# anand-12/botorch

Hardware: AMD Instinct MI355X
Metric: acq-evals/sec (q x restarts x MC), qEI forward (higher is better)
Workload: dtype f64; 1 GPU; C3 qEI forward: SingleTaskGP n=4096 d=6, q=16, 512 restarts/GPU, 512 Sobol MC samples, best_f = max(Y) - 1.5; n=4096, d=6, q=16, restarts_per_gpu=512, mc=512, parallelism=restart-sharded x1

## Files before the change

botorch_amd/_lib.py:

```python
from __future__ import annotations

import ctypes
import os
from ctypes import POINTER, c_double, c_int, c_int64, c_void_p

_HERE = os.path.dirname(os.path.abspath(__file__))
LIB_PATH = os.path.join(_HERE, "libbotorch_amd.so")

BO_OK, BO_ERR_ARG, BO_ERR_HIP, BO_ERR_NOT_PSD, BO_ERR_NAN = 0, 1, 2, 3, 4
RBF, MATERN52 = 0, 1
GEMM_LOWER_C, GEMM_A_LOWER, GEMM_B_UPPER, GEMM_A_UPPER, GEMM_B_LOWER = 1, 2, 4, 8, 16
QMC_POSTERIOR, QMC_QEI, QMC_QNEI, QMC_CHOL, QMC_QLOGEI, QMC_QLOGNEI = 0, 1, 2, 3, 4, 5
QMC_QSR, QMC_QPI, QMC_QUCB = 6, 7, 8
LOG_MODES = (QMC_QLOGEI, QMC_QLOGNEI)
MC_MODES = (QMC_QEI, QMC_QNEI) + LOG_MODES + (QMC_QSR, QMC_QPI, QMC_QUCB)
ABI_VERSION = 12
RT_ROWMAJOR, RT_BLOCKED = 0, 1

_P = c_void_p

_SIGNATURES = {
    "bo_last_error": (ctypes.c_char_p, []),
    "bo_version": (c_int, []),
    "bo_probe_mfma_f64_layout": (c_int, [_P, _P]),
# ... 48 lines not shown
    "bo_post_w_members_work": (c_int, [c_int, c_int, c_int, c_int64, POINTER(c_int64)]),
    "bo_post_w_split_members": (c_int, [c_int, _P, c_int64, _P, c_int, c_int, c_int64, _P, _P, _P]),
    "bo_post_w_dx_work": (c_int, [c_int, c_int, c_int64, POINTER(c_int64)]),
    "bo_post_w_dx": (c_int, [c_int, _P, c_int64, _P, c_int, c_int, c_int, c_int64, _P, _P, _P, _P,
                             _P, _P, c_double, c_double, _P, _P, _P]),
    "bo_ainv": (c_int, [_P, c_int64, c_int64, _P, _P, _P]),
    "bo_sym_lower": (c_int, [_P, c_int64, c_int64, _P]),
    "bo_post_kxt_rows": (c_int, [c_int, _P, c_int, c_int, c_int, _P, _P, c_int64, c_double, _P,
                                 _P, _P]),
    "bo_post_quad_plan": (c_int, [c_int64, c_int, c_int64, POINTER(c_int)]),
    "bo_post_small_plan": (c_int, [c_int64, c_int, c_int64, POINTER(c_int)]),
    "bo_post_set_wide": (c_int, [c_int]),
    "bo_post_wide_applies": (c_int, [c_int64, c_int, c_int64, c_int, c_int, c_int, POINTER(c_int)]),
    "bo_post_wide_schedule": (c_int, [c_int, c_int, c_int, c_int, POINTER(c_int), POINTER(c_int),
                                      _P]),
    "bo_post_small": (c_int, [_P, c_int64, c_int, c_int64, _P, c_int64, _P, _P, _P, _P, _P]),
    "bo_post_small_batched": (c_int, [c_int, _P, _P, _P, _P, _P, _P, c_int64, c_int, c_int64,
                                      c_int64, _P]),
    "bo_pinned_alloc": (c_int, [c_int64, POINTER(c_void_p), POINTER(c_void_p)]),
    "bo_pinned_free": (c_int, [c_void_p]),
    "bo_qmc_finalize_members": (c_int, [c_int, c_int, c_int, c_int, _P, _P, _P, c_int64, _P, _P, _P,
                                        _P, c_int, c_double, _P, _P, _P, _P, c_int, _P, _P, _P,
                                        c_int, c_int64, _P, c_int64, _P]),
    "bo_post_kxt_rows_members": (c_int, [c_int, c_int, _P, c_int, c_int, c_int, _P, _P, _P, c_int64,
                                         _P, _P, _P]),
    "bo_post_members_work": (c_int, [c_int, c_int64, c_int, c_int64, POINTER(c_int64)]),
    "bo_post_partials_members": (c_int, [c_int, _P, _P, _P, _P, _P, _P, _P, c_int64, c_int,
                                         c_int64, c_int64, _P, _P]),
    "bo_post_quad": (c_int, [_P, _P, c_int64, _P, c_int64, c_int, c_int64, _P, _P, _P]),
    "bo_post_split_table": (c_int, [c_int64, c_int, c_int64, c_int, _P, c_int, _P, c_int,
# ... 231 lines not shown
    "bo_qmc_feas_v": QmcFeasArgs, "bo_qmc_feas_backward_v": QmcFeasArgs,
    "bo_kg_v": KgArgs, "bo_kg_backward_v": KgArgs,
    "bo_paths_eval_v": PathsArgs, "bo_paths_eval_backward_v": PathsArgs,
    "bo_jes_v": JesArgs, "bo_jes_backward_v": JesArgs,
    "bo_mes_v": MesArgs, "bo_mes_backward_v": MesArgs,
    "bo_gibbon_v": GibbonArgs, "bo_gibbon_backward_v": GibbonArgs,
    "bo_mv_quantiles_v": MvQuantilesArgs,
    "bo_nipv_gram_v": NipvArgs, "bo_nipv_gram_backward_v": NipvArgs,
    "bo_bald_v": BaldArgs, "bo_bald_backward_v": BaldArgs,
    "bo_analytic_v": AnalyticArgs, "bo_analytic_backward_v": AnalyticArgs,
    "bo_saas_potential_v": SaasPotentialArgs,
    "bo_lbfgs_step_v": LbfgsStepArgs, "bo_lbfgsb_step_v": LbfgsbArgs,
}
for _name, _cls in RECORD_ENTRIES.items():
    _SIGNATURES[_name] = (c_int, [POINTER(_cls), _P])
_SIGNATURES["bo_saas_potential_work"] = (c_int, [c_int64, c_int, c_int64, POINTER(c_int64)])
_SIGNATURES["bo_struct_size"] = (c_int64, [ctypes.c_char_p])
_SIGNATURES["bo_post_backward_jobs"] = (c_int, [c_int, POINTER(POINTER(PostBackwardArgs)), _P, _P])
ARG_RECORDS = {"BoPostPartialsArgs": PostPartialsArgs, "BoQmcFinalizeArgs": QmcFinalizeArgs,
               "BoQmcBackwardArgs": QmcBackwardArgs, "BoPostBackwardArgs": PostBackwardArgs,
               "BoQehviArgs": QehviArgs, "BoQehviFeasArgs": QehviFeasArgs,
               "BoQlogehviArgs": QlogehviArgs, "BoQmcFeasArgs": QmcFeasArgs, "BoKgArgs": KgArgs,
               "BoPathsArgs": PathsArgs, "BoJesArgs": JesArgs, "BoMesArgs": MesArgs,
               "BoGibbonArgs": GibbonArgs, "BoMvQuantilesArgs": MvQuantilesArgs,
               "BoNipvArgs": NipvArgs, "BoBaldArgs": BaldArgs, "BoAnalyticArgs": AnalyticArgs,
               "BoSaasPotentialArgs": SaasPotentialArgs,
               "BoLbfgsStepArgs": LbfgsStepArgs, "BoLbfgsbArgs": LbfgsbArgs}

_lib = None

# ... 62 lines not shown
```

botorch_amd/csrc/abi_structs.cpp:

```cpp
#include <cstdio>
#include <string>

#include "../../include/botorch_amd.h"

void bo_set_error(const char* fmt, ...);

namespace {

template <class T>
bool header_ok(const T* a, const char* name) {
  if (!a) {
    bo_set_error("%s: null argument struct", name);
    return false;
  }
  if (a->struct_size != sizeof(T) || a->abi_version != BO_ABI_VERSION) {
    bo_set_error("%s: struct size %u / ABI %u, library expects %zu / %d", name, a->struct_size,
                 a->abi_version, sizeof(T), BO_ABI_VERSION);
    return false;
  }
  return true;
}

}

// ... 35 lines not shown
  X(PostPartials) X(QmcFinalize) X(QmcBackward) X(PostBackward) X(Qehvi) X(QehviFeas)          \
  X(Qlogehvi) X(QmcFeas) X(Kg) X(Paths) X(Jes) X(Mes) X(Gibbon) X(MvQuantiles) X(Nipv) X(Bald) \
  X(Analytic) X(SaasPotential) X(LbfgsStep) X(Lbfgsb)

extern "C" {

#define BO_ENTRY(entry, record)                                         \
  int bo_##entry##_impl(const Bo##record##Args* a, void* stream);       \
  int bo_##entry##_v(const Bo##record##Args* a, void* stream) {         \
    if (!header_ok(a, "bo_" #entry "_v")) return BO_ERR_ARG;            \
    return bo_##entry##_impl(a, stream);                                \
  }
BO_RECORD_ENTRIES(BO_ENTRY)
#undef BO_ENTRY

int64_t bo_struct_size(const char* name) {
  const std::string s = name ? name : "";
#define BO_SIZE(record) \
  if (s == "Bo" #record "Args") return sizeof(Bo##record##Args);
  BO_RECORDS(BO_SIZE)
#undef BO_SIZE
  return -1;
}

}
```

botorch_amd/csrc/post.hip:

```cpp
#include "common.h"
#include "post_wide_sched.h"

#include <algorithm>
#include <atomic>
#include <cstdlib>
#include <map>
#include <mutex>
#include <tuple>
#include <vector>

namespace {

constexpr int PC = 128;
constexpr int PI = 128;
constexpr int PK = 16;
constexpr int PLD = 144;
constexpr int DP = 8;
constexpr int kSlots = 512;
constexpr int kTileDoubles = 32 * 64;
#ifndef KXT_K
#define KXT_K 16
#endif

template <int KIND, int ND>
// ... 553 lines not shown
      m += __shfl_xor(m, 16);
      m += __shfl_xor(m, 32);
      if (lane < 16) mpart[(int64_t)ci * nrows_pad + row0 + lane] = m;
    }
    }
  }
  }
}

#ifndef BO_POSTW_PRIO
#define BO_POSTW_PRIO 0
#endif
__global__ __launch_bounds__(512, 2) void post_partials_wide_kernel(
    int n, const double* __restrict__ U, int64_t ldu, const double* __restrict__ beta, int nC,
    int nI, double* __restrict__ Spart, double* __restrict__ mpart, double* __restrict__ Rt,
    const double* __restrict__ Kt, int rt_blk) {
  constexpr int SS = postw::kSS, NU = postw::kNU;
  __shared__ __attribute__((aligned(16))) double Us[postw::kStages][SS * PK][PLD];
  const int bid = blockIdx.x;
  const int xcd = bid & 7;
  const int slot = bid >> 3;
  const int tt = (slot >> 5) * 8 + xcd;
  const int w = slot & 31;
  const int nIG = nI >> 3;
  const int p = tt / nIG;
  if (p >= (nC >> 4)) return;
  const int ci_long = ((nC >> 3) - 1 - p) * 8 + 7 - (w & 7);
  const int ci_short = p * 8 + (w & 7);
  const int i0 = ((tt % nIG) * 4 + (w >> 3)) * (2 * PI);
  const int tid = threadIdx.x;
  const int lane = tid & 63;
  const int wave = __builtin_amdgcn_readfirstlane(tid >> 6);
  const bool late = postw::kLag > 0 && wave >= 4;
#if BO_POSTW_PRIO
  if (__builtin_amdgcn_readfirstlane(threadIdx.x) >= 256) __builtin_amdgcn_s_setprio(1);
#endif
  const int64_t ldk = (int64_t)nI * PI;
  const int nrows16 = nI * (PI / 16);
  const int lag = postw::lag_of(late);

  for (int sidx = 0; sidx < 2; ++sidx) {
    const int ci = sidx == 0 ? ci_long : ci_short;
    const int c0 = ci * PC;
    const int kend = min(n, c0 + PC);
// ... 152 lines not shown
          const int c = c0 + ct * 16 + mfma_row(lane, r);
          m = fma(acc[ct][it][r], (c < n) ? beta[c] : 0.0, m);
        }
      m += __shfl_xor(m, 16);
      m += __shfl_xor(m, 32);
      if (lane < 16) mpart[(int64_t)ci * nrows_pad + row0 + lane] = m;
    }
  }
}

struct RowsFromX {
  const double* X;
  const double* ls;
  int B, q, d, Qp;
  double* Xq_out;
};

struct KxtMembers {
  const double* ls[8];
  const double* Xt[8];
  double os[8];
  double* Xq[8];
  double* Kt[8];
  int nm;
};

template <int KIND, int ND, int KK = KXT_K, bool FROMX = false>
__global__ __launch_bounds__(256) void kxt_build_kernel(const double* __restrict__ Xq, int nrows,
                                                        const double* __restrict__ Xt, int n,
                                                        int np, int nrows_pad, double outputscale,
                                                        double* __restrict__ Kt,
                                                        RowsFromX rx = RowsFromX{},
                                                        KxtMembers km = KxtMembers{}) {
  if (km.nm > 0) {
    const int m = blockIdx.z;
    rx.ls = km.ls[m];
    rx.Xq_out = km.Xq[m];
    Xt = km.Xt[m];
    outputscale = km.os[m];
    Kt = km.Kt[m];
  }
  const int i = blockIdx.x * 256 + threadIdx.x;
  const int k0 = blockIdx.y * KK;
  const bool iv = i < nrows;
  double xi[ND];
  if constexpr (FROMX) {
    const int b = i / rx.Qp, a = i - (i / rx.Qp) * rx.Qp;
    const bool real = iv && b < rx.B && a < rx.q;
#pragma unroll
    for (int t = 0; t < ND; ++t)
      xi[t] = (real && t < rx.d) ? rx.X[((int64_t)b * rx.q + a) * rx.d + t] / rx.ls[t] : 0.0;
    if (blockIdx.y == 0 && i < nrows_pad) {
#pragma unroll
      for (int t = 0; t < DP; ++t)
        rx.Xq_out[(int64_t)i * DP + t] =
            (real && t < rx.d) ? rx.X[((int64_t)b * rx.q + a) * rx.d + t] / rx.ls[t] : 0.0;
    }
  } else {
#pragma unroll
    for (int t = 0; t < ND; ++t) xi[t] = iv ? Xq[(int64_t)i * DP + t] : 0.0;
  }
  if (i >= nrows_pad) return;
#pragma unroll 4
  for (int kk = 0; kk < KK; ++kk) {
    const int k = k0 + kk;
    if (k < np) Kt[(int64_t)k * nrows_pad + i] = eval_kernel_row<KIND, ND>(xi, Xt, n, k, outputscale, iv);
  }
}

__global__ __launch_bounds__(256) void post_splitk_reduce_kernel(
    const double* __restrict__ work, const int4* __restrict__ red, int n, int nI,
    const double* __restrict__ beta_all, double* __restrict__ Spart_all,
    double* __restrict__ mpart_all, double* __restrict__ Rt_all, PostMembers pm = PostMembers{}) {
  __shared__ double part[3][32][64];
  const int4 r4 = red[blockIdx.x / (PI / 16)];
  const int sub = blockIdx.x % (PI / 16);
  const int ci = r4.x & 0xffffff, rt = r4.y * (PI / 16) + sub;
  const int mem = r4.x >> 24;
  const bool memb = pm.nm > 0;
  const double* beta = memb ? pm.beta[mem] : beta_all;
  double* Spart = memb ? pm.Spart[mem] : Spart_all;
// ... 363 lines not shown
#ifndef BO_POST_WIDE_DEFAULT
#define BO_POST_WIDE_DEFAULT 1
#endif
static std::atomic<int>& wide_mode() {
  static std::atomic<int> m{[] {
    const char* e = std::getenv("BO_POST_WIDE");
    const int v = e ? std::atoi(e) : 0;
    return v >= -1 && v <= 1 ? v : 0;
  }()};
  return m;
}
static bool wide_applies(int nC, int nI, int kc_len, bool cross, bool pre) {
  const int mode = wide_mode().load();
  if (mode < 0 || (mode == 0 && !BO_POST_WIDE_DEFAULT)) return false;
  return kc_len == 0 && !cross && pre && nI > 0 && nC % 16 == 0 && nI % 8 == 0 && paired_enabled();
}

struct SplitPlan {
  std::vector<int4> segs, red;
  std::vector<int> wg_off;
  int nchunks = 0, max_segs = 0;
  int64_t max_steps = 0;
};

static int sk_min_share() {
  static const int v = [] {
    const char* e = std::getenv("BO_SK_MIN_SHARE");
    const int x = e ? std::atoi(e) : 4;
    return x >= 1 ? x : 4;
  }();
// ... 420 lines not shown
  BO_CHECK_ARG(X && lengthscale && Xt_scaled && outputscale && Xq && Kt,
               "bo_post_kxt_rows_members: null pointer");
  KxtMembers km{};
  km.nm = nm;
  for (int m = 0; m < nm; ++m) {
    BO_CHECK_ARG(lengthscale[m] && Xt_scaled[m] && Xq[m] && Kt[m], "bo_post_kxt_rows_members: null buffer");
    km.ls[m] = lengthscale[m];
    km.Xt[m] = Xt_scaled[m];
    km.os[m] = outputscale[m];
    km.Xq[m] = Xq[m];
    km.Kt[m] = Kt[m];
  }
  const int np = nC * PC;
  const int nrows = B * Qp;
  hipStream_t st = as_stream(stream);
  const RowsFromX rx{X, lengthscale[0], B, q, d, Qp, Xq[0]};
  const bool small = ceil_div(nrows_pad, 256) * ceil_div(np, KXT_K) * nm < 1024;
  const int kk = small ? kxt_small_k() : KXT_K;
  const dim3 grid((unsigned)ceil_div(nrows_pad, 256), (unsigned)ceil_div(np, kk), (unsigned)nm);
#define BO_KXTM_K(KIND, ND, K)                                                                 \
  kxt_build_kernel<KIND, ND, K, true><<<grid, 256, 0, st>>>(nullptr, nrows, Xt_scaled[0], (int)n, \
                                                            np, nrows_pad, outputscale[0], Kt[0], rx, km)
#define BO_KXTM(KIND, ND)                  \
  switch (kk) {                            \
    case 1: BO_KXTM_K(KIND, ND, 1); break; \
    case 2: BO_KXTM_K(KIND, ND, 2); break; \
    case 4: BO_KXTM_K(KIND, ND, 4); break; \
    case 8: BO_KXTM_K(KIND, ND, 8); break; \
    default: BO_KXTM_K(KIND, ND, KXT_K); break; \
  }
#define BO_KXTM_D(KIND)                      \
// ... 6 lines not shown
    case 6: BO_KXTM(KIND, 6); break;         \
    default: BO_KXTM(KIND, 8); break;        \
  }
  if (kind == BO_RBF) {
    BO_KXTM_D(BO_RBF)
  } else {
    BO_KXTM_D(BO_MATERN52)
  }
#undef BO_KXTM_D
#undef BO_KXTM
#undef BO_KXTM_K
  BO_LAUNCH_CHECK();
  return BO_OK;
}

int bo_post_kxt_rows(int kind, const double* X, int B, int q, int d, const double* lengthscale,
                     const double* Xt_scaled, int64_t n, double outputscale, double* Xq, double* Kt,
                     void* stream) {
  BO_CHECK_ARG(kind == BO_RBF || kind == BO_MATERN52, "bad kernel kind %d", kind);
  BO_CHECK_ARG(d >= 1 && d <= DP, "fused posterior kernel supports 1 <= d <= %d", DP);
  int Qp, nrows_pad, nC;
  int s = bo_post_geometry(B, q, n, &Qp, &nrows_pad, &nC);
  if (s) return s;
  if (nrows_pad == 0) return BO_OK;
  BO_CHECK_ARG(X && lengthscale && Xt_scaled && Xq && Kt, "bo_post_kxt_rows: null buffer");
  const int np = nC * PC;
  const int nrows = B * Qp;
  hipStream_t st = as_stream(stream);
  const RowsFromX rx{X, lengthscale, B, q, d, Qp, Xq};
  const bool small = ceil_div(nrows_pad, 256) * ceil_div(np, KXT_K) < 1024;
  const int kk = small ? kxt_small_k() : KXT_K;
  const dim3 grid((unsigned)ceil_div(nrows_pad, 256), (unsigned)ceil_div(np, kk));
#define BO_KXTR_K(KIND, ND, K)                                                                 \
  kxt_build_kernel<KIND, ND, K, true><<<grid, 256, 0, st>>>(nullptr, nrows, Xt_scaled, (int)n,  \
                                                            np, nrows_pad, outputscale, Kt, rx)
#define BO_KXTR(KIND, ND)                  \
  switch (kk) {                            \
    case 1: BO_KXTR_K(KIND, ND, 1); break; \
    case 2: BO_KXTR_K(KIND, ND, 2); break; \
    case 4: BO_KXTR_K(KIND, ND, 4); break; \
    case 8: BO_KXTR_K(KIND, ND, 8); break; \
    default: BO_KXTR_K(KIND, ND, KXT_K); break; \
  }
#define BO_KXTR_D(KIND)                      \
  switch (d) {                               \
    case 1: BO_KXTR(KIND, 1); break;         \
    case 2: BO_KXTR(KIND, 2); break;         \
    case 3: BO_KXTR(KIND, 3); break;         \
    case 4: BO_KXTR(KIND, 4); break;         \
    case 5: BO_KXTR(KIND, 5); break;         \
    case 6: BO_KXTR(KIND, 6); break;         \
    default: BO_KXTR(KIND, 8); break;        \
  }
  if (kind == BO_RBF) {
    BO_KXTR_D(BO_RBF)
  } else {
    BO_KXTR_D(BO_MATERN52)
  }
#undef BO_KXTR_D
#undef BO_KXTR
#undef BO_KXTR_K
  BO_LAUNCH_CHECK();
  return BO_OK;
}

int bo_post_partials_impl(const BoPostPartialsArgs* a, void* stream) {
  const int kc_len = a->kc_len;
  const int64_t n = a->n;
  const bool blocked = a->rt_layout == BO_RT_BLOCKED;
  BO_CHECK_ARG(a->rt_layout == BO_RT_ROWMAJOR || (blocked && kc_len == 0 && !a->Qc),
               "rt_layout %d: the blocked R^T is stored by one-pass grids without a cross term",
               a->rt_layout);
  BO_CHECK_ARG(a->Qc == nullptr || (kc_len == 0 && a->rq >= 1 && a->rq <= 16 && a->ldq >= n &&
                                    a->Cx != nullptr),
               "cross term: one-pass only, 1 <= rq <= 16 rows (got %d), ldq >= n, Cx given", a->rq);
  BO_CHECK_ARG(a->kind == BO_RBF || a->kind == BO_MATERN52, "bad kernel kind %d", a->kind);
  BO_CHECK_ARG(a->ldu % 2 == 0 && a->ldu >= ceil_div(n, PC) * PC, "U leading dim %lld too small",
               (long long)a->ldu);
  if (a->B == 0) return BO_OK;
  const bool pre = a->Kt != nullptr;
  BO_CHECK_ARG(kc_len == 0 || kc_len == -1 || (kc_len > 0 && kc_len % PK == 0),
// ... 9 lines not shown
                          ? ((nC % 16 == 0 && paired_enabled()) ? 2 : 1) : 0;
  DevPlan* plan = nullptr;
  if (kc_len != 0) {
    s = device_plan(nC, nI, (int)n, kc_len, &plan);
    if (s) return s;
    BO_CHECK_ARG(plan->nchunks == 0 || a->work != nullptr, "split plan needs a workspace of %lld doubles",
                 (long long)plan->nchunks * PI * PC);
  }
  const int64_t blocks = kc_len != 0    ? plan->W
                         : grouped == 2 ? 512 * (int64_t)ceil_div((nC / 16) * (nI / 8), 8)
                         : grouped      ? 512 * (int64_t)ceil_div((nC / 8) * (nI / 8), 8)
                                        : 8 * ceil_div(nC, 8) * (int64_t)nI;
  const int4* segs = plan ? plan->segs : nullptr;
  const int* wg_off = plan ? plan->wg_off : nullptr;
  hipStream_t st = as_stream(stream);
  if (wide_applies(nC, nI, kc_len, a->Qc != nullptr, pre)) {
    const int64_t wblocks = 256 * (int64_t)ceil_div((nC / 16) * (nI / 8), 8);
    post_partials_wide_kernel<<<(unsigned)wblocks, 512, 0, st>>>(
        (int)n, a->U, a->ldu, a->beta, nC, nI, a->Spart, a->mpart, a->Rt, a->Kt, blocked);
    BO_LAUNCH_CHECK();
    return BO_OK;
  }
#define BO_POST_GO(KIND, ND, SPL, CRS, PRE_)                                                \
  post_partials_kernel<KIND, ND, SPL, CRS, PRE_><<<(unsigned)blocks, 256, 0, st>>>(          \
      a->Xq, nrows, a->Xt_scaled, (int)n, a->U, a->ldu, a->beta, a->outputscale, nC, nI,    \
      a->Spart, a->mpart, a->Rt, segs, wg_off, a->work, a->Qc, a->rq, a->ldq, a->Cx, a->Kt, \
      grouped, FusedDx{}, blocked)
#define BO_POST_LAUNCH(KIND, ND)                                                            \
  if (kc_len != 0) {                                                                        \
    if (pre) BO_POST_GO(KIND, ND, true, false, true);                                       \
    else BO_POST_GO(KIND, ND, true, false, false);                                          \
  } else if (a->Qc != nullptr) {                                                            \
    if (pre) BO_POST_GO(KIND, ND, false, true, true);                                     \
    else BO_POST_GO(KIND, ND, false, true, false);                                          \
// ... 16 lines not shown
  } else {
    BO_POST_DISPATCH_D(BO_MATERN52)
  }
#undef BO_POST_DISPATCH_D
#undef BO_POST_LAUNCH
#undef BO_POST_GO
  BO_LAUNCH_CHECK();
  if (plan && plan->nred > 0) {
    post_splitk_reduce_kernel<<<(unsigned)(plan->nred * (PI / 16)), 256, 0, st>>>(
        a->work, plan->red, (int)n, nI, a->beta, a->Spart, a->mpart, a->Rt);
    BO_LAUNCH_CHECK();
  }
  return BO_OK;
}

int bo_post_set_wide(int mode) {
  BO_CHECK_ARG(mode >= -1 && mode <= 1, "bo_post_set_wide: mode %d (-1, 0 or 1)", mode);
  wide_mode().store(mode);
  return BO_OK;
}

int bo_post_wide_applies(int64_t B, int q, int64_t n, int kc_len, int has_cross, int has_kt,
                         int* out) {
  int Qp, nrows_pad, nC;
  int s = bo_post_geometry(B, q, n, &Qp, &nrows_pad, &nC);
  if (s) return s;
  *out = wide_applies(nC, nrows_pad / PI, kc_len, has_cross != 0, has_kt != 0) ? 1 : 0;
  return BO_OK;
}

int bo_post_wide_schedule(int nsteps, int half, int rev, int cap, int* n_barriers, int* n_events,
                          int* events) {
  BO_CHECK_ARG(nsteps >= 1 && (half == 0 || half == 1) && n_barriers && n_events,
               "bo_post_wide_schedule: nsteps %d, half %d", nsteps, half);
  const bool late = half == 1;
  const int lag = postw::lag_of(late);
  int ne = 0;
  auto emit = [&](int j, int kind, int step, int slice) {
    if (events && ne < cap) {
      int* e = events + 6 * (int64_t)ne;
      e[0] = j; e[1] = kind; e[2] = step; e[3] = slice; e[4] = postw::stage_of_step(step);
      e[5] = postw::walk_k0(step, nsteps, rev != 0, PK);
// ... 253 lines not shown
```

botorch_amd/csrc/torch/bo_torch.cpp:

```cpp
#include <ATen/ATen.h>
#include <c10/hip/HIPStream.h>
#include <hip/hip_runtime_api.h>
#include <torch/library.h>

#include <algorithm>
#include <array>
#include <deque>
#include <atomic>
#include <mutex>
#include <unordered_map>
#include <utility>
#include <vector>

#include "../../../include/botorch_amd.h"

namespace {

void ck(int rc, const char* what) {
  TORCH_CHECK(rc == BO_OK, "botorch_amd ", what, ": ", bo_last_error());
}
void hk(hipError_t e, const char* what) {
  TORCH_CHECK(e == hipSuccess, "botorch_amd ", what, ": ", hipGetErrorString(e));
}
const double* cp(const at::Tensor& t) { return t.defined() && t.numel() ? t.data_ptr<double>() : nullptr; }
// ... 101 lines not shown
  ck(bo_ladder_status(info.data_ptr<int>(), jitter.data_ptr<double>(), info.numel(),
                      L.slot[mine].dev, stream), "ladder_status");
  publish_slot(L, mine, stream);
  return prev;
}

std::mutex g_time_mu;
bool g_time_on = false;
std::vector<std::pair<hipEvent_t, hipEvent_t>> g_time_ev;

hipEvent_t timing_event(void* stream) {
  hipEvent_t e;
  hk(hipEventCreate(&e), "hipEventCreate");
  hk(hipEventRecord(e, static_cast<hipStream_t>(stream)), "hipEventRecord");
  return e;
}

std::vector<at::Tensor> qmc_acq_impl(
    const at::Tensor& X, const at::Tensor& Xt_scaled, const at::Tensor& U, const at::Tensor& Linv,
    const at::Tensor& beta, const at::Tensor& lengthscale, const at::Tensor& Z,
    const c10::optional<at::Tensor>& best_f_s, int64_t kind, int64_t mode, int64_t n,
    double outputscale, double constant, double ymean, double ystd, double best_f, bool fat,
    double tau_relu, double tau_max, bool need_grad, int64_t kxt_cap, bool defer_ladder,
    const c10::optional<at::Tensor>& Ainv, const c10::optional<at::Tensor>& alpha, bool lean,
    const c10::optional<at::Tensor>& cap_status = c10::nullopt,
    const c10::optional<at::Tensor>& cap_count = c10::nullopt) {
  check_f64(X, "X");
  check_f64(Xt_scaled, "Xt_scaled");
  check_f64(U, "U");
  check_f64(beta, "beta");
// ... 40 lines not shown
  const int64_t o_xq = o_work + (kc ? al2(std::max<int64_t>(we, 1)) : 0);
  const int64_t o_info = o_xq + (own_xq ? 0 : al2(int64_t(nrows) * 8));
  const int64_t o_jit = o_info + (lean ? al2((B + 1) / 2) : 0);
  const int64_t total = o_jit + (lean ? al2(B) : 0);
  auto ws = at::empty({std::max<int64_t>(total, 2)}, f64);
  double* w = ws.data_ptr<double>();
  double* Spart = w + o_spart;
  double* mpart = w + o_mpart;
  double* Kt = kxt ? w + o_kt : nullptr;
  double* work = kc ? w + o_work : nullptr;
  at::Tensor Xq_t = own_xq ? at::empty({nrows, 8}, f64) : at::Tensor();
  double* Xq = own_xq ? Xq_t.data_ptr<double>() : w + o_xq;
  at::Tensor Rt = need_grad ? at::empty({int64_t(nC) * 128, nrows}, f64) : at::Tensor();
  int rt_layout = BO_RT_ROWMAJOR;

  if (kxt) {
    ck(bo_post_kxt_rows(int(kind), X.data_ptr<double>(), B, q, d, lengthscale.data_ptr<double>(),
                        Xt_scaled.data_ptr<double>(), n, outputscale, Xq, Kt, st), "post_kxt_rows");
  } else {
    ck(bo_prepare_rows(X.data_ptr<double>(), B, q, d, lengthscale.data_ptr<double>(), Xq, st),
       "prepare_rows");
  }
  hipEvent_t t0 = nullptr;
  {
    std::lock_guard<std::mutex> lk(g_time_mu);
    if (g_time_on) t0 = timing_event(st);
  }
  if (npairs > 0) {
    ck(bo_post_quad(Kt, Ainv->data_ptr<double>(), np, alpha->data_ptr<double>(), B, q, n, Spart,
                    mpart, st), "post_quad");
  } else if (nsmall > 0) {
// ... 14 lines not shown
    pa.ldu = np;
    pa.beta = beta.data_ptr<double>();
    pa.outputscale = outputscale;
    pa.Spart = Spart;
    pa.mpart = mpart;
    pa.Rt = mp(Rt);
    pa.kc_len = kc;
    pa.work = work;
    pa.Kt = Kt;
    if (need_grad) {
      int64_t wdx = 0;
      ck(bo_post_w_dx_work(B, q, n, &wdx), "post_w_dx_work");
      rt_layout = (wdx > 0 && kc == 0) ? BO_RT_BLOCKED : BO_RT_ROWMAJOR;
      pa.rt_layout = rt_layout;
    }
    ck(bo_post_partials_v(&pa, st), "post_partials");
  }
  if (t0) {
    std::lock_guard<std::mutex> lk(g_time_mu);
    g_time_ev.emplace_back(t0, timing_event(st));
  }

  auto acq = at::empty({B}, f64);
  at::Tensor info, jit;
  if (!lean) {
    info = at::empty({B}, X.options().dtype(at::kInt));
    jit = at::empty({B}, f64);
  }
  int* info_p = lean ? reinterpret_cast<int*>(w + o_info) : info.data_ptr<int>();
  double* jit_p = lean ? w + o_jit : jit.data_ptr<double>();
  at::Tensor mean = need_grad ? at::empty({B, q}, f64) : at::Tensor();
// ... 865 lines not shown
        "Tensor? Ainv=None, Tensor? alpha=None) -> Tensor[]");
  m.def("qmc_acq_eager(Tensor X, Tensor Xt_scaled, Tensor U, Tensor beta, Tensor lengthscale, "
        "Tensor Z, Tensor? best_f_s, int kind, int mode, int n, float outputscale, float constant, "
        "float ymean, float ystd, float best_f, bool fat, float tau_relu, float tau_max, "
        "int kxt_cap, Tensor? Ainv=None, Tensor? alpha=None, Tensor? cap_status=None, "
        "Tensor? cap_count=None) -> Tensor[]");
  m.def("qmc_acq_backward_native(Tensor dacq, Tensor acq, Tensor mean, Tensor L, Tensor Z, "
        "Tensor? best_f_s, Tensor Xq, Tensor Rt, Tensor Linv, Tensor U, Tensor Xt_scaled, "
        "Tensor alpha, Tensor lengthscale, int kind, int mode, int d, int n, float outputscale, "
        "float ystd, float best_f, bool fat, float tau_relu, float tau_max) -> Tensor");
  m.def("ladder_defer(Tensor info, Tensor jitter) -> Tensor");
  m.def("ladder_poll(int device) -> Tensor", &ladder_poll);
  m.def("post_timing(bool on) -> ()", &post_timing);
  m.def("post_timing_read() -> Tensor", &post_timing_read);
  m.def("last_backward_route() -> int", &last_backward_route);
  m.def("pinned_status() -> Tensor", &pinned_status);
}

TORCH_LIBRARY_IMPL(bo, CUDA, m) {
  m.impl("qmc_acq_native", &qmc_acq_native);
  m.impl("qmc_acq_eager", &qmc_acq_eager);
  m.impl("qmc_acq_backward_native", &qmc_acq_backward_native);
  m.impl("ladder_defer", &ladder_defer);
  m.impl("qehvi_members_eager", &qehvi_members_eager);
  m.impl("jes_native", &jes_native);
  m.impl("jes_backward_native", &jes_backward_native);
  m.impl("mes_native", &mes_native);
  m.impl("mes_backward_native", &mes_backward_native);
  m.impl("gibbon_native", &gibbon_native);
  m.impl("gibbon_backward_native", &gibbon_backward_native);
// ... 6 lines not shown
```

botorch_amd/kernels.py:

```python
from __future__ import annotations

import collections
import ctypes
import functools
import math
import os
from dataclasses import dataclass
from typing import Optional

import torch
from torch.quasirandom import SobolEngine

from . import _lib
from ._lib import check, lib

DP = 8
KXT_MAX_BYTES = int(os.environ.get("BO_KXT_MAX_BYTES", 4 << 30))
_KXT_CAP = {}


def kxt_cap(device: torch.device) -> int:
    idx = device.index if device.index is not None else torch.cuda.current_device()
    if idx not in _KXT_CAP:
        _KXT_CAP[idx] = min(KXT_MAX_BYTES, torch.cuda.get_device_properties(idx).total_memory // 16)
# ... 623 lines not shown
                              n=cache.n, U=cache.U, ldu=cache.np, beta=cache.beta,
                              outputscale=cache.outputscale, Spart=Spart, mpart=mpart, Rt=Rt,
                              kc_len=kc_len, work=work, Qc=cross if Cx is not None else None,
                              rq=cross.shape[0] if Cx is not None else 0,
                              ldq=cross.shape[1] if Cx is not None else 0, Cx=Cx, Kt=Kt,
                              rt_layout=int(rt_layout))
    check(lib().bo_post_partials_v(ctypes.byref(a), st), "post_partials")
    if TIMING_HOOK is not None:
        TIMING_HOOK("post_partials_end")
    if Rt is not None and rt_layout == _lib.RT_BLOCKED:
        Rt = Rt.view(nC * 8, nrows_pad // 16, 256)
    return PostPartials(B, q, Qp, nrows_pad, nC, Xq, Spart, mpart, Rt,
                        Cx.sum(dim=0) if Cx is not None else None)


def qmc_finalize(cache: GPCache, pp: PostPartials, mode: int, ymean: float, ystd: float,
                 Z: Optional[torch.Tensor] = None, best_f: float = 0.0,
                 best_f_s: Optional[torch.Tensor] = None, want_mean=True, want_cov=True,
                 want_L=False, max_tries=CHOLESKY_MAX_TRIES, jitter0=CHOLESKY_JITTER_F64,
                 T: Optional[torch.Tensor] = None, F: Optional[torch.Tensor] = None,
                 log_params: Optional[tuple] = None, mean_out: Optional[torch.Tensor] = None,
                 L_out: Optional[torch.Tensor] = None, status=None):
    dev = pp.Xq.device
    B, q = pp.B, pp.q
    f64 = dict(dtype=torch.float64, device=dev)
    for t, shp in ((mean_out, (B, q)), (L_out, (B, q, q))):
        if t is not None and (tuple(t.shape) != shp or not t.is_contiguous() or t.dtype != torch.float64):
            raise ValueError(f"qmc_finalize: output buffer must be contiguous fp64 {shp}")
    mean = (mean_out if mean_out is not None else torch.empty(B, q, **f64)) if want_mean else None
    cov = torch.empty(B, q, q, **f64) if want_cov else None
# ... 1687 lines not shown
```

include/botorch_amd.h:

```cpp
#ifndef BOTORCH_AMD_H
#define BOTORCH_AMD_H

#include <stdint.h>

#ifdef __cplusplus
extern "C" {
#endif

#define BO_ABI_VERSION 12

#define BO_OK 0
#define BO_ERR_ARG 1
#define BO_ERR_HIP 2
#define BO_ERR_NOT_PSD 3
#define BO_ERR_NAN 4

#define BO_KIND_RBF 0
#define BO_KIND_MATERN52 1

#define BO_GEMM_LOWER_C 1
#define BO_GEMM_A_LOWER 2
#define BO_GEMM_B_UPPER 4
#define BO_GEMM_A_UPPER 8
#define BO_GEMM_B_LOWER 16
// ... 131 lines not shown

int bo_post_w_dx_work(int B, int q, int64_t n, int64_t* work_elems);
int bo_post_w_dx(int kind, const double* Linv, int64_t ldl, const double* Rt, int B, int q, int d,
                 int64_t n, const double* Xq, const double* Xt_scaled, const double* alpha,
                 const double* dmean, const double* dcov, const double* lengthscale,
                 double outputscale, double ystd, double* work, double* dX, void* stream);

int bo_post_split_plan(int64_t B, int q, int64_t n, int slots, int* kc_len,
                       int64_t* work_elems);
int bo_post_split_work(int64_t B, int q, int64_t n, int kc_len, int64_t* work_elems);
int bo_post_set_wide(int mode);
int bo_post_wide_applies(int64_t B, int q, int64_t n, int kc_len, int has_cross, int has_kt,
                         int* out);
int bo_post_wide_schedule(int nsteps, int half, int rev, int cap, int* n_barriers, int* n_events,
                          int* events);

int bo_post_small_plan(int64_t B, int q, int64_t n, int* nparts);
int bo_post_small(const double* Kt, int64_t B, int q, int64_t n, const double* U, int64_t ldu,
                  const double* beta, double* Spart, double* mpart, double* Rt, void* stream);
int bo_post_small_batched(int nm, const double* const* Kt, const double* const* U,
                          const double* const* beta, double* const* Spart, double* const* mpart,
                          double* const* Rt, int64_t B, int q, int64_t n, int64_t ldu,
                          void* stream);
int bo_post_members_work(int nm, int64_t B, int q, int64_t n, int64_t* work_elems);
int bo_post_kxt_rows_members(int nm, int kind, const double* X, int B, int q, int d,
                             const double* const* lengthscale, const double* const* Xt_scaled,
                             const double* outputscale, int64_t n, double* const* Xq,
                             double* const* Kt, void* stream);
int bo_post_partials_members(int nm, const double* const* Kt, const double* const* U,
                             const double* const* beta, double* const* Spart, double* const* mpart,
// ... 67 lines not shown
  int64_t n;
  const double* U;
  int64_t ldu;
  const double* beta;
  double outputscale;
  double *Spart, *mpart, *Rt;
  int32_t kc_len, rq;
  double* work;
  const double* Qc;
  int64_t ldq;
  double* Cx;
  const double* Kt;
  int32_t rt_layout, _pad;
} BoPostPartialsArgs;
int bo_post_partials_v(const BoPostPartialsArgs* a, void* stream);

typedef struct BoQmcFinalizeArgs {
  BO_STRUCT_HEADER;
  int32_t kind, mode, B, q;
  const double *Xq, *Spart, *mpart;
  int64_t n;
  double outputscale, constant, ymean, ystd;
  const double* Z;
  int32_t S, max_tries;
  double best_f;
  const double* best_f_s;
  double jitter0;
  double *acq, *mean_out, *cov_out, *L_out;
  int* info_out;
  double* jitter_out;
// ... 302 lines not shown
```

Measured before the change: 2.011 billion acq-evals/s.

## Split posterior row groups and overlap second-half Kxt build on side stream

In the qEI forward path, the rows are split into two halves. The Kxt kernel-matrix build for the second half runs on a non-blocking side stream with a persistent CU-sized grid, while the wide partials kernel processes the first half on the main stream. The aim is to hide Kxt construction behind the partials compute instead of running the two serially. The cost is extra launches, event synchronisation, a global mutex around the split streams, and the background kernel competing with partials for CUs.

```diff
diff --git a/botorch_amd/_lib.py b/botorch_amd/_lib.py
--- a/botorch_amd/_lib.py
+++ b/botorch_amd/_lib.py
@@ -86,6 +86,11 @@
     "bo_post_wide_applies": (c_int, [c_int64, c_int, c_int64, c_int, c_int, c_int, POINTER(c_int)]),
     "bo_post_wide_schedule": (c_int, [c_int, c_int, c_int, c_int, POINTER(c_int), POINTER(c_int),
                                       _P]),
+    "bo_post_kxt_rows_range": (c_int, [c_int, _P, c_int, c_int, c_int, _P, _P, c_int64, c_double, _P,
+                                       _P, c_int, c_int, c_int, _P]),
+    "bo_post_set_rowsplit": (c_int, [c_int]),
+    "bo_post_rowsplit_applies": (c_int, [c_int64, c_int, c_int64, c_int, c_int, c_int,
+                                         POINTER(c_int)]),
     "bo_post_small": (c_int, [_P, c_int64, c_int, c_int64, _P, c_int64, _P, _P, _P, _P, _P]),
     "bo_post_small_batched": (c_int, [c_int, _P, _P, _P, _P, _P, _P, c_int64, c_int, c_int64,
                                       c_int64, _P]),
@@ -347,6 +352,7 @@
 }
 for _name, _cls in RECORD_ENTRIES.items():
     _SIGNATURES[_name] = (c_int, [POINTER(_cls), _P])
+_SIGNATURES["bo_post_partials_rows"] = (c_int, [POINTER(PostPartialsArgs), c_int, c_int, _P])
 _SIGNATURES["bo_saas_potential_work"] = (c_int, [c_int64, c_int, c_int64, POINTER(c_int64)])
 _SIGNATURES["bo_struct_size"] = (c_int64, [ctypes.c_char_p])
 _SIGNATURES["bo_post_backward_jobs"] = (c_int, [c_int, POINTER(POINTER(PostBackwardArgs)), _P, _P])
diff --git a/botorch_amd/csrc/abi_structs.cpp b/botorch_amd/csrc/abi_structs.cpp
--- a/botorch_amd/csrc/abi_structs.cpp
+++ b/botorch_amd/csrc/abi_structs.cpp
@@ -73,6 +73,12 @@
 BO_RECORD_ENTRIES(BO_ENTRY)
 #undef BO_ENTRY
 
+int bo_post_partials_rows_impl(const BoPostPartialsArgs* a, int rg0, int nrg, void* stream);
+int bo_post_partials_rows(const BoPostPartialsArgs* a, int rg0, int nrg, void* stream) {
+  if (!header_ok(a, "bo_post_partials_rows")) return BO_ERR_ARG;
+  return bo_post_partials_rows_impl(a, rg0, nrg, stream);
+}
+
 int64_t bo_struct_size(const char* name) {
   const std::string s = name ? name : "";
 #define BO_SIZE(record) \
diff --git a/botorch_amd/csrc/post.hip b/botorch_amd/csrc/post.hip
--- a/botorch_amd/csrc/post.hip
+++ b/botorch_amd/csrc/post.hip
@@ -591,7 +591,7 @@
 __global__ __launch_bounds__(512, 2) void post_partials_wide_kernel(
     int n, const double* __restrict__ U, int64_t ldu, const double* __restrict__ beta, int nC,
     int nI, double* __restrict__ Spart, double* __restrict__ mpart, double* __restrict__ Rt,
-    const double* __restrict__ Kt, int rt_blk) {
+    const double* __restrict__ Kt, int rt_blk, int rg0, int nrg) {
   constexpr int SS = postw::kSS, NU = postw::kNU;
   __shared__ __attribute__((aligned(16))) double Us[postw::kStages][SS * PK][PLD];
   const int bid = blockIdx.x;
@@ -599,12 +599,11 @@
   const int slot = bid >> 3;
   const int tt = (slot >> 5) * 8 + xcd;
   const int w = slot & 31;
-  const int nIG = nI >> 3;
-  const int p = tt / nIG;
+  const int p = tt / nrg;
   if (p >= (nC >> 4)) return;
   const int ci_long = ((nC >> 3) - 1 - p) * 8 + 7 - (w & 7);
   const int ci_short = p * 8 + (w & 7);
-  const int i0 = ((tt % nIG) * 4 + (w >> 3)) * (2 * PI);
+  const int i0 = ((rg0 + tt % nrg) * 4 + (w >> 3)) * (2 * PI);
   const int tid = threadIdx.x;
   const int lane = tid & 63;
   const int wave = __builtin_amdgcn_readfirstlane(tid >> 6);
@@ -787,7 +786,24 @@
   const double* ls;
   int B, q, d, Qp;
   double* Xq_out;
+  int row0, row1;
 };
+
+template <int ND>
+__device__ __forceinline__ void scaled_row_from_x(const RowsFromX& rx, int i, bool iv, bool store,
+                                                  double (&xi)[ND]) {
+  const int b = i / rx.Qp, a = i - (i / rx.Qp) * rx.Qp;
+  const bool real = iv && b < rx.B && a < rx.q;
+#pragma unroll
+  for (int t = 0; t < ND; ++t)
+    xi[t] = (real && t < rx.d) ? rx.X[((int64_t)b * rx.q + a) * rx.d + t] / rx.ls[t] : 0.0;
+  if (store) {
+#pragma unroll
+    for (int t = 0; t < DP; ++t)
+      rx.Xq_out[(int64_t)i * DP + t] =
+          (real && t < rx.d) ? rx.X[((int64_t)b * rx.q + a) * rx.d + t] / rx.ls[t] : 0.0;
+  }
+}
 
 struct KxtMembers {
   const double* ls[8];
@@ -813,31 +829,46 @@
     outputscale = km.os[m];
     Kt = km.Kt[m];
   }
-  const int i = blockIdx.x * 256 + threadIdx.x;
+  const int i = (FROMX ? rx.row0 : 0) + blockIdx.x * 256 + threadIdx.x;
+  const int iend = FROMX ? rx.row1 : nrows_pad;
   const int k0 = blockIdx.y * KK;
   const bool iv = i < nrows;
   double xi[ND];
   if constexpr (FROMX) {
-    const int b = i / rx.Qp, a = i - (i / rx.Qp) * rx.Qp;
-    const bool real = iv && b < rx.B && a < rx.q;
-#pragma unroll
-    for (int t = 0; t < ND; ++t)
-      xi[t] = (real && t < rx.d) ? rx.X[((int64_t)b * rx.q + a) * rx.d + t] / rx.ls[t] : 0.0;
-    if (blockIdx.y == 0 && i < nrows_pad) {
-#pragma unroll
-      for (int t = 0; t < DP; ++t)
-        rx.Xq_out[(int64_t)i * DP + t] =
-            (real && t < rx.d) ? rx.X[((int64_t)b * rx.q + a) * rx.d + t] / rx.ls[t] : 0.0;
-    }
+    scaled_row_from_x<ND>(rx, i, iv, blockIdx.y == 0 && i < iend, xi);
   } else {
 #pragma unroll
     for (int t = 0; t < ND; ++t) xi[t] = iv ? Xq[(int64_t)i * DP + t] : 0.0;
   }
-  if (i >= nrows_pad) return;
+  if (i >= iend) return;
 #pragma unroll 4
   for (int kk = 0; kk < KK; ++kk) {
     const int k = k0 + kk;
     if (k < np) Kt[(int64_t)k * nrows_pad + i] = eval_kernel_row<KIND, ND>(xi, Xt, n, k, outputscale, iv);
+  }
+}
+
+#ifndef BO_KXT_BG_WGS
+#define BO_KXT_BG_WGS 1
+#endif
+template <int KIND, int ND>
+__global__ __launch_bounds__(256) void kxt_build_bg_kernel(int nrows, const double* __restrict__ Xt,
+                                                           int n, int np, int nrows_pad,
+                                                           double outputscale,
+                                                           double* __restrict__ Kt, RowsFromX rx,
+                                                           int ksegs, int kseg_len) {
+  const int nblk = (rx.row1 - rx.row0 + 255) / 256;
+  for (int u = blockIdx.x; u < nblk * ksegs; u += gridDim.x) {
+    const int blk = u / ksegs, seg = u - blk * ksegs;
+    const int i = rx.row0 + blk * 256 + threadIdx.x;
+    const bool iv = i < nrows;
+    double xi[ND];
+    scaled_row_from_x<ND>(rx, i, iv, seg == 0 && i < rx.row1, xi);
+    if (i >= rx.row1) continue;
+    const int kend = min(np, (seg + 1) * kseg_len);
+#pragma unroll 2
+    for (int k = seg * kseg_len; k < kend; ++k)
+      Kt[(int64_t)k * nrows_pad + i] = eval_kernel_row<KIND, ND>(xi, Xt, n, k, outputscale, iv);
   }
 }
 
@@ -1231,6 +1262,25 @@
   const int mode = wide_mode().load();
   if (mode < 0 || (mode == 0 && !BO_POST_WIDE_DEFAULT)) return false;
   return kc_len == 0 && !cross && pre && nI > 0 && nC % 16 == 0 && nI % 8 == 0 && paired_enabled();
+}
+
+#ifndef BO_POST_ROWSPLIT_DEFAULT
+#define BO_POST_ROWSPLIT_DEFAULT 1
+#endif
+static std::atomic<int>& rowsplit_mode() {
+  static std::atomic<int> m{[] {
+    const char* e = std::getenv("BO_POST_ROWSPLIT");
+    const int v = e ? std::atoi(e) : 0;
+    return v >= -1 && v <= 1 ? v : 0;
+  }()};
+  return m;
+}
+static bool rowsplit_applies(int nC, int nI, int kc_len, bool cross, bool pre) {
+  const int mode = rowsplit_mode().load();
+  if (mode < 0 || !wide_applies(nC, nI, kc_len, cross, pre)) return false;
+  const int nrg = nI / 8;
+  if (mode == 1) return nrg >= 2;
+  return BO_POST_ROWSPLIT_DEFAULT && nrg % 2 == 0 && ((nC / 16) * (nI / 16)) % 8 == 0;
 }
 
 struct SplitPlan {
@@ -1681,7 +1731,7 @@
   const int np = nC * PC;
   const int nrows = B * Qp;
   hipStream_t st = as_stream(stream);
-  const RowsFromX rx{X, lengthscale[0], B, q, d, Qp, Xq[0]};
+  const RowsFromX rx{X, lengthscale[0], B, q, d, Qp, Xq[0], 0, nrows_pad};
   const bool small = ceil_div(nrows_pad, 256) * ceil_div(np, KXT_K) * nm < 1024;
   const int kk = small ? kxt_small_k() : KXT_K;
   const dim3 grid((unsigned)ceil_div(nrows_pad, 256), (unsigned)ceil_div(np, kk), (unsigned)nm);
@@ -1718,33 +1768,60 @@
   return BO_OK;
 }
 
-int bo_post_kxt_rows(int kind, const double* X, int B, int q, int d, const double* lengthscale,
-                     const double* Xt_scaled, int64_t n, double outputscale, double* Xq, double* Kt,
-                     void* stream) {
-  BO_CHECK_ARG(kind == BO_RBF || kind == BO_MATERN52, "bad kernel kind %d", kind);
-  BO_CHECK_ARG(d >= 1 && d <= DP, "fused posterior kernel supports 1 <= d <= %d", DP);
-  int Qp, nrows_pad, nC;
-  int s = bo_post_geometry(B, q, n, &Qp, &nrows_pad, &nC);
-  if (s) return s;
-  if (nrows_pad == 0) return BO_OK;
-  BO_CHECK_ARG(X && lengthscale && Xt_scaled && Xq && Kt, "bo_post_kxt_rows: null buffer");
+static int device_cu_count(int* out) {
+  static std::mutex mu;
+  static std::map<int, int> cus;
+  int dev = 0;
+  BO_HIP(hipGetDevice(&dev));
+  std::lock_guard<std::mutex> lk(mu);
+  auto it = cus.find(dev);
+  if (it == cus.end()) {
+    int v = 0;
+    BO_HIP(hipDeviceGetAttribute(&v, hipDeviceAttributeMultiprocessorCount, dev));
+    it = cus.emplace(dev, std::max(v, 1)).first;
+  }
+  *out = it->second;
+  return BO_OK;
+}
+
+static int kxt_rows_launch(int kind, const double* X, int B, int q, int d, const double* lengthscale,
+                           const double* Xt_scaled, int64_t n, double outputscale, double* Xq,
+                           double* Kt, int Qp, int nrows_pad, int nC, int row0, int row1,
+                           bool background, void* stream) {
   const int np = nC * PC;
   const int nrows = B * Qp;
   hipStream_t st = as_stream(stream);
-  const RowsFromX rx{X, lengthscale, B, q, d, Qp, Xq};
-  const bool small = ceil_div(nrows_pad, 256) * ceil_div(np, KXT_K) < 1024;
+  const RowsFromX rx{X, lengthscale, B, q, d, Qp, Xq, row0, row1};
+  const int nblk = (int)ceil_div(row1 - row0, 256);
+  const bool small = nblk * ceil_div(np, KXT_K) < 1024;
   const int kk = small ? kxt_small_k() : KXT_K;
-  const dim3 grid((unsigned)ceil_div(nrows_pad, 256), (unsigned)ceil_div(np, kk));
+  const dim3 grid((unsigned)nblk, (unsigned)ceil_div(np, kk));
+  int bg_grid = 0, ksegs = 1, kseg_len = np;
+  if (background) {
+    int cus = 0;
+    const int s = device_cu_count(&cus);
+    if (s) return s;
+    bg_grid = cus * BO_KXT_BG_WGS;
+    ksegs = (int)std::min<int64_t>(std::max<int64_t>(1, ceil_div(bg_grid, nblk)), np / KXT_K);
+    kseg_len = (int)(ceil_div(ceil_div(np, ksegs), KXT_K) * KXT_K);
+    ksegs = (int)ceil_div(np, kseg_len);
+    bg_grid = std::min(bg_grid, nblk * ksegs);
+  }
 #define BO_KXTR_K(KIND, ND, K)                                                                 \
   kxt_build_kernel<KIND, ND, K, true><<<grid, 256, 0, st>>>(nullptr, nrows, Xt_scaled, (int)n,  \
                                                             np, nrows_pad, outputscale, Kt, rx)
-#define BO_KXTR(KIND, ND)                  \
-  switch (kk) {                            \
-    case 1: BO_KXTR_K(KIND, ND, 1); break; \
-    case 2: BO_KXTR_K(KIND, ND, 2); break; \
-    case 4: BO_KXTR_K(KIND, ND, 4); break; \
-    case 8: BO_KXTR_K(KIND, ND, 8); break; \
-    default: BO_KXTR_K(KIND, ND, KXT_K); break; \
+#define BO_KXTR(KIND, ND)                                                                      \
+  if (background) {                                                                            \
+    kxt_build_bg_kernel<KIND, ND><<<(unsigned)bg_grid, 256, 0, st>>>(                          \
+        nrows, Xt_scaled, (int)n, np, nrows_pad, outputscale, Kt, rx, ksegs, kseg_len);        \
+  } else {                                                                                     \
+    switch (kk) {                                                                              \
+      case 1: BO_KXTR_K(KIND, ND, 1); break;                                                   \
+      case 2: BO_KXTR_K(KIND, ND, 2); break;                                                   \
+      case 4: BO_KXTR_K(KIND, ND, 4); break;                                                   \
+      case 8: BO_KXTR_K(KIND, ND, 8); break;                                                   \
+      default: BO_KXTR_K(KIND, ND, KXT_K); break;                                              \
+    }                                                                                          \
   }
 #define BO_KXTR_D(KIND)                      \
   switch (d) {                               \
@@ -1768,7 +1845,42 @@
   return BO_OK;
 }
 
-int bo_post_partials_impl(const BoPostPartialsArgs* a, void* stream) {
+int bo_post_kxt_rows(int kind, const double* X, int B, int q, int d, const double* lengthscale,
+                     const double* Xt_scaled, int64_t n, double outputscale, double* Xq, double* Kt,
+                     void* stream) {
+  BO_CHECK_ARG(kind == BO_RBF || kind == BO_MATERN52, "bad kernel kind %d", kind);
+  BO_CHECK_ARG(d >= 1 && d <= DP, "fused posterior kernel supports 1 <= d <= %d", DP);
+  int Qp, nrows_pad, nC;
+  int s = bo_post_geometry(B, q, n, &Qp, &nrows_pad, &nC);
+  if (s) return s;
+  if (nrows_pad == 0) return BO_OK;
+  BO_CHECK_ARG(X && lengthscale && Xt_scaled && Xq && Kt, "bo_post_kxt_rows: null buffer");
+  return kxt_rows_launch(kind, X, B, q, d, lengthscale, Xt_scaled, n, outputscale, Xq, Kt, Qp,
+                         nrows_pad, nC, 0, nrows_pad, false, stream);
+}
+
+int bo_post_kxt_rows_range(int kind, const double* X, int B, int q, int d,
+                           const double* lengthscale, const double* Xt_scaled, int64_t n,
+                           double outputscale, double* Xq, double* Kt, int row0, int nrows_range,
+                           int background, void* stream) {
+  BO_CHECK_ARG(kind == BO_RBF || kind == BO_MATERN52, "bad kernel kind %d", kind);
+  BO_CHECK_ARG(d >= 1 && d <= DP, "fused posterior kernel supports 1 <= d <= %d", DP);
+  int Qp, nrows_pad, nC;
+  int s = bo_post_geometry(B, q, n, &Qp, &nrows_pad, &nC);
+  if (s) return s;
+  BO_CHECK_ARG(row0 >= 0 && nrows_range >= 0 && row0 % PI == 0 && nrows_range % PI == 0 &&
+                   (int64_t)row0 + nrows_range <= nrows_pad,
+               "bo_post_kxt_rows_range: rows %d + %d of %d (whole %d-row tiles inside the batch)",
+               row0, nrows_range, nrows_pad, PI);
+  BO_CHECK_ARG(background == 0 || background == 1, "bo_post_kxt_rows_range: background %d", background);
+  if (nrows_range == 0) return BO_OK;
+  BO_CHECK_ARG(X && lengthscale && Xt_scaled && Xq && Kt, "bo_post_kxt_rows_range: null buffer");
+  return kxt_rows_launch(kind, X, B, q, d, lengthscale, Xt_scaled, n, outputscale, Xq, Kt, Qp,
+                         nrows_pad, nC, row0, row0 + nrows_range, background != 0, stream);
+}
+
+static int post_partials_launch(const BoPostPartialsArgs* a, bool rows, int rg0, int nrg,
+                                void* stream) {
   const int kc_len = a->kc_len;
   const int64_t n = a->n;
   const bool blocked = a->rt_layout == BO_RT_BLOCKED;
@@ -1808,10 +1920,19 @@
   const int4* segs = plan ? plan->segs : nullptr;
   const int* wg_off = plan ? plan->wg_off : nullptr;
   hipStream_t st = as_stream(stream);
-  if (wide_applies(nC, nI, kc_len, a->Qc != nullptr, pre)) {
-    const int64_t wblocks = 256 * (int64_t)ceil_div((nC / 16) * (nI / 8), 8);
+  const bool wide = wide_applies(nC, nI, kc_len, a->Qc != nullptr, pre);
+  BO_CHECK_ARG(!rows || (wide && rg0 >= 0 && nrg >= 0 && rg0 + nrg <= nI / 8),
+               "bo_post_partials_rows: row groups %d + %d of %d (8-wave route %s)", rg0, nrg,
+               wide ? nI / 8 : 0, wide ? "taken" : "not taken at this shape");
+  if (wide) {
+    if (!rows) {
+      rg0 = 0;
+      nrg = nI / 8;
+    }
+    if (nrg == 0) return BO_OK;
+    const int64_t wblocks = 256 * (int64_t)ceil_div((nC / 16) * nrg, 8);
     post_partials_wide_kernel<<<(unsigned)wblocks, 512, 0, st>>>(
-        (int)n, a->U, a->ldu, a->beta, nC, nI, a->Spart, a->mpart, a->Rt, a->Kt, blocked);
+        (int)n, a->U, a->ldu, a->beta, nC, nI, a->Spart, a->mpart, a->Rt, a->Kt, blocked, rg0, nrg);
     BO_LAUNCH_CHECK();
     return BO_OK;
   }
@@ -1858,6 +1979,14 @@
   return BO_OK;
 }
 
+int bo_post_partials_impl(const BoPostPartialsArgs* a, void* stream) {
+  return post_partials_launch(a, false, 0, 0, stream);
+}
+
+int bo_post_partials_rows_impl(const BoPostPartialsArgs* a, int rg0, int nrg, void* stream) {
+  return post_partials_launch(a, true, rg0, nrg, stream);
+}
+
 int bo_post_set_wide(int mode) {
   BO_CHECK_ARG(mode >= -1 && mode <= 1, "bo_post_set_wide: mode %d (-1, 0 or 1)", mode);
   wide_mode().store(mode);
@@ -1870,6 +1999,22 @@
   int s = bo_post_geometry(B, q, n, &Qp, &nrows_pad, &nC);
   if (s) return s;
   *out = wide_applies(nC, nrows_pad / PI, kc_len, has_cross != 0, has_kt != 0) ? 1 : 0;
+  return BO_OK;
+}
+
+int bo_post_set_rowsplit(int mode) {
+  BO_CHECK_ARG(mode >= -1 && mode <= 1, "bo_post_set_rowsplit: mode %d (-1, 0 or 1)", mode);
+  rowsplit_mode().store(mode);
+  return BO_OK;
+}
+
+int bo_post_rowsplit_applies(int64_t B, int q, int64_t n, int kc_len, int has_cross, int has_kt,
+                             int* out) {
+  BO_CHECK_ARG(out != nullptr, "bo_post_rowsplit_applies: null out");
+  int Qp, nrows_pad, nC;
+  int s = bo_post_geometry(B, q, n, &Qp, &nrows_pad, &nC);
+  if (s) return s;
+  *out = rowsplit_applies(nC, nrows_pad / PI, kc_len, has_cross != 0, has_kt != 0) ? 1 : 0;
   return BO_OK;
 }
 
diff --git a/botorch_amd/csrc/torch/bo_torch.cpp b/botorch_amd/csrc/torch/bo_torch.cpp
--- a/botorch_amd/csrc/torch/bo_torch.cpp
+++ b/botorch_amd/csrc/torch/bo_torch.cpp
@@ -139,6 +139,49 @@
   hk(hipEventCreate(&e), "hipEventCreate");
   hk(hipEventRecord(e, static_cast<hipStream_t>(stream)), "hipEventRecord");
   return e;
+}
+
+struct SplitStreams {
+  hipStream_t side = nullptr;
+  hipEvent_t e1 = nullptr, e2 = nullptr;
+};
+std::mutex g_split_mu;
+std::unordered_map<int, SplitStreams> g_split;
+
+SplitStreams& split_streams_for(int dev) {
+  auto& ss = g_split[dev];
+  if (!ss.side) {
+    int cur = 0;
+    hk(hipGetDevice(&cur), "hipGetDevice");
+    if (cur != dev) hk(hipSetDevice(dev), "hipSetDevice");
+    hipStream_t side = nullptr;
+    hipEvent_t e1 = nullptr, e2 = nullptr;
+    const hipError_t a = hipStreamCreateWithFlags(&side, hipStreamNonBlocking);
+    const hipError_t b = hipEventCreateWithFlags(&e1, hipEventDisableTiming);
+    const hipError_t c = hipEventCreateWithFlags(&e2, hipEventDisableTiming);
+    if (cur != dev) (void)hipSetDevice(cur);
+    hk(a, "hipStreamCreate");
+    hk(b, "hipEventCreate");
+    hk(c, "hipEventCreate");
+    ss.e1 = e1;
+    ss.e2 = e2;
+    ss.side = side;
+  }
+  return ss;
+}
+
+enum { BO_FWD_SINGLE = 0, BO_FWD_ROWSPLIT = 1 };
+std::atomic<int> g_last_fwd_route{BO_FWD_SINGLE};
+
+int64_t last_forward_route() { return g_last_fwd_route.load(); }
+
+bool stream_is_capturing(void* st) {
+  hipStreamCaptureStatus cs = hipStreamCaptureStatusNone;
+  if (hipStreamIsCapturing(static_cast<hipStream_t>(st), &cs) != hipSuccess) {
+    (void)hipGetLastError();
+    return true;
+  }
+  return cs != hipStreamCaptureStatusNone;
 }
 
 std::vector<at::Tensor> qmc_acq_impl(
@@ -209,7 +252,27 @@
   at::Tensor Rt = need_grad ? at::empty({int64_t(nC) * 128, nrows}, f64) : at::Tensor();
   int rt_layout = BO_RT_ROWMAJOR;
 
-  if (kxt) {
+  bool split = false;
+  if (!need_grad && kxt && npairs == 0 && nsmall == 0 && B > 0) {
+    int ap = 0;
+    ck(bo_post_rowsplit_applies(B, q, n, kc, 0, 1, &ap), "post_rowsplit_applies");
+    split = ap != 0 && !stream_is_capturing(st);
+  }
+  g_last_fwd_route.store(split ? BO_FWD_ROWSPLIT : BO_FWD_SINGLE);
+  const int nrg = nrows / 1024, rg_a = nrg / 2, rg_b = nrg - rg_a;
+  auto kxt_groups = [&](int g0, int ng, int background, void* s) {
+    return bo_post_kxt_rows_range(int(kind), X.data_ptr<double>(), B, q, d,
+                                  lengthscale.data_ptr<double>(), Xt_scaled.data_ptr<double>(), n,
+                                  outputscale, Xq, Kt, g0 * 1024, ng * 1024, background, s);
+  };
+  std::unique_lock<std::mutex> split_lk(g_split_mu, std::defer_lock);
+  SplitStreams* ss = nullptr;
+  if (split) {
+    split_lk.lock();
+    ss = &split_streams_for(dev);
+    ck(kxt_groups(0, rg_a, 0, st), "post_kxt_rows_range");
+    hk(hipEventRecord(ss->e1, static_cast<hipStream_t>(st)), "hipEventRecord");
+  } else if (kxt) {
     ck(bo_post_kxt_rows(int(kind), X.data_ptr<double>(), B, q, d, lengthscale.data_ptr<double>(),
                         Xt_scaled.data_ptr<double>(), n, outputscale, Xq, Kt, st), "post_kxt_rows");
   } else {
@@ -254,7 +317,23 @@
       rt_layout = (wdx > 0 && kc == 0) ? BO_RT_BLOCKED : BO_RT_ROWMAJOR;
       pa.rt_layout = rt_layout;
     }
-    ck(bo_post_partials_v(&pa, st), "post_partials");
+    if (split) {
+      hipStream_t s0 = static_cast<hipStream_t>(st);
+      const int rc_a = bo_post_partials_rows(&pa, 0, rg_a, st);
+      const hipError_t he_w = hipStreamWaitEvent(ss->side, ss->e1, 0);
+      const int rc_k = he_w == hipSuccess ? kxt_groups(rg_a, rg_b, 1, ss->side) : BO_OK;
+      const hipError_t he_r = hipEventRecord(ss->e2, ss->side);
+      const hipError_t he_j = he_r == hipSuccess ? hipStreamWaitEvent(s0, ss->e2, 0) : he_r;
+      if (he_j != hipSuccess) (void)hipStreamSynchronize(ss->side);
+      ck(rc_a, "post_partials_rows");
+      hk(he_w, "hipStreamWaitEvent");
+      ck(rc_k, "post_kxt_rows_range");
+      hk(he_j, "hipStreamWaitEvent");
+      ck(bo_post_partials_rows(&pa, rg_a, rg_b, st), "post_partials_rows");
+      split_lk.unlock();
+    } else {
+      ck(bo_post_partials_v(&pa, st), "post_partials");
+    }
   }
   if (t0) {
     std::lock_guard<std::mutex> lk(g_time_mu);
@@ -1150,6 +1229,7 @@
   m.def("post_timing(bool on) -> ()", &post_timing);
   m.def("post_timing_read() -> Tensor", &post_timing_read);
   m.def("last_backward_route() -> int", &last_backward_route);
+  m.def("last_forward_route() -> int", &last_forward_route);
   m.def("pinned_status() -> Tensor", &pinned_status);
 }
 
diff --git a/botorch_amd/kernels.py b/botorch_amd/kernels.py
--- a/botorch_amd/kernels.py
+++ b/botorch_amd/kernels.py
@@ -661,6 +661,40 @@
                         Cx.sum(dim=0) if Cx is not None else None)
 
 
+def set_post_rowsplit(mode: int) -> None:
+    check(lib().bo_post_set_rowsplit(int(mode)), "post_set_rowsplit")
+
+
+def post_rowsplit_applies(B: int, q: int, n: int, kc_len: int = 0, cross: bool = False,
+                          kt: bool = True) -> int:
+    out = ctypes.c_int(-1)
+    check(lib().bo_post_rowsplit_applies(B, q, n, kc_len, int(cross), int(kt), ctypes.byref(out)),
+          "post_rowsplit_applies")
+    return out.value
+
+
+def post_kxt_rows_range(cache: GPCache, X: torch.Tensor, Xq: torch.Tensor, Kt: torch.Tensor,
+                        row0: int, nrows_range: int, background: bool = False) -> None:
+    B, q, d = X.shape
+    check(lib().bo_post_kxt_rows_range(cache.kind, _p(X.contiguous()), B, q, d,
+                                       _p(cache.lengthscale), _p(cache.Xt_scaled), cache.n,
+                                       cache.outputscale, _p(Xq), _p(Kt), int(row0),
+                                       int(nrows_range), int(background), _stream(_dev(X))),
+          "post_kxt_rows_range")
+
+
+def post_partials_rows(cache: GPCache, B: int, q: int, d: int, Xq: torch.Tensor, Kt: torch.Tensor,
+                       Spart: torch.Tensor, mpart: torch.Tensor, Rt: Optional[torch.Tensor],
+                       rt_layout: int, rg0: int, nrg: int) -> None:
+    a = _lib.PostPartialsArgs(kind=cache.kind, B=B, q=q, d=d, Xq=Xq, Xt_scaled=cache.Xt_scaled,
+                              n=cache.n, U=cache.U, ldu=cache.np, beta=cache.beta,
+                              outputscale=cache.outputscale, Spart=Spart, mpart=mpart, Rt=Rt,
+                              kc_len=0, work=None, Qc=None, rq=0, ldq=0, Cx=None, Kt=Kt,
+                              rt_layout=int(rt_layout))
+    check(lib().bo_post_partials_rows(ctypes.byref(a), int(rg0), int(nrg), _stream(_dev(Xq))),
+          "post_partials_rows")
+
+
 def qmc_finalize(cache: GPCache, pp: PostPartials, mode: int, ymean: float, ystd: float,
                  Z: Optional[torch.Tensor] = None, best_f: float = 0.0,
                  best_f_s: Optional[torch.Tensor] = None, want_mean=True, want_cov=True,
diff --git a/include/botorch_amd.h b/include/botorch_amd.h
--- a/include/botorch_amd.h
+++ b/include/botorch_amd.h
@@ -169,6 +169,14 @@
                          int* out);
 int bo_post_wide_schedule(int nsteps, int half, int rev, int cap, int* n_barriers, int* n_events,
                           int* events);
+
+int bo_post_kxt_rows_range(int kind, const double* X, int B, int q, int d,
+                           const double* lengthscale, const double* Xt_scaled, int64_t n,
+                           double outputscale, double* Xq, double* Kt, int row0, int nrows_range,
+                           int background, void* stream);
+int bo_post_set_rowsplit(int mode);
+int bo_post_rowsplit_applies(int64_t B, int q, int64_t n, int kc_len, int has_cross, int has_kt,
+                             int* out);
 
 int bo_post_small_plan(int64_t B, int q, int64_t n, int* nparts);
 int bo_post_small(const double* Kt, int64_t B, int q, int64_t n, const double* U, int64_t ldu,
@@ -266,6 +274,7 @@
   int32_t rt_layout, _pad;
 } BoPostPartialsArgs;
 int bo_post_partials_v(const BoPostPartialsArgs* a, void* stream);
+int bo_post_partials_rows(const BoPostPartialsArgs* a, int rg0, int nrg, void* stream);
 
 typedef struct BoQmcFinalizeArgs {
   BO_STRUCT_HEADER;
```

After: 2.027 billion acq-evals/s, median of 6. About the same (+0.8%).
